# ccalantzis/BRDF

Measured on AMD Instinct MI355X. Metric: BRDF residual-evals/sec (1 M samples, Ward 3-param), whole job; rel-err vs CPU levmar in `parity`, higher is better.
Workload: dtype f64

## Files before the change

### brdf_amd/csrc/brdf_models.h

```cpp
#pragma once

#include <math.h>

#include "lm_machine.h"

namespace brdf {

constexpr double kPi = 3.1415926535897932384626433832795;

enum ModelId : int { MODEL_PHONG = 0, MODEL_BLINN_PHONG = 1, MODEL_WARD = 2, MODEL_COUNT = 3 };

struct Lin {
  double a, b;
};
struct Nl {
  double u0, u1;
};
struct Prep {
  double q1, q2;
};

template <int MODEL>
struct BrdfModel;

// ... 115 lines not shown
  Nl n0;
  Lin lp[kM];
  Lin lm[kM];
  Nl np2, nm2;
  double dinv[kM];
  Lin lq;
  Nl nq;
  Lin lk[kMaxCand];
  Nl nk[kMaxCand];
  double dp[kM], dp_l2, scal;
  double an[2];
  int central, ncand, analytic;

  LM_HD void build(const Request<kM> &r, bool need_base = true, bool analytic_jac = false) {
    ncand = 0;
    analytic = analytic_jac ? 1 : 0;
    if (r.kind == RQ_EVAL_MULTI) {
      ncand = r.nk;
      for (int j = 0; j < kMaxCand; ++j)
        if (j < r.nk) {
          lk[j] = Mdl::lin(r.pk[j]);
          nk[j] = Mdl::nl(r.pk[j]);
        }
      return;
    }
    if (r.kind != RQ_DIF_UPDATE && (need_base || r.kind != RQ_DIF_TRIAL)) {
      l0 = Mdl::lin(r.p);
      n0 = Mdl::nl(r.p);
    }
    central = r.central;
    scal = r.scal;
    dp_l2 = r.dp_l2;
    for (int j = 0; j < kM; ++j) dp[j] = r.dp[j];
    if (r.kind == RQ_JAC && analytic_jac) {
      Mdl::an_scalars(r.p, an);
    } else if (r.kind == RQ_JAC || r.kind == RQ_DIF_JAC) {
      for (int j = 0; j < kM; ++j) {
        double pp[kM] = {r.p[0], r.p[1], r.p[2]};
        pp[j] = r.p[j] + r.d[j];
        lp[j] = Mdl::lin(pp);
        if (j == kM - 1) np2 = Mdl::nl(pp);
        double pm[kM] = {r.p[0], r.p[1], r.p[2]};
        pm[j] = r.p[j] - r.d[j];
        lm[j] = Mdl::lin(pm);
        if (j == kM - 1) nm2 = Mdl::nl(pm);
        dinv[j] = (r.central ? 0.5 : 1.0) / r.d[j];
      }
    }
    if (r.kind == RQ_DIF_TRIAL) {
      lq = Mdl::lin(r.q);
      nq = Mdl::nl(r.q);
    }
  }
};

template <int MODEL, bool FAST, class U>
LM_HD double model_value(const U &u, double c0, const Prep &q) {
  using Mdl = BrdfModel<MODEL>;
  return Mdl::combine(u.l0, c0, Mdl::template shape<FAST>(u.n0, c0, q));
}

template <int MODEL, bool FAST>
LM_HD double model_value_k(const PassUniforms<MODEL> &u, int j, double c0, const Prep &q) {
  using Mdl = BrdfModel<MODEL>;
  return Mdl::combine(u.lk[j], c0, Mdl::template shape<FAST>(u.nk[j], c0, q));
}

template <int MODEL, bool FAST, class U>
LM_HD double model_value_q(const U &u, double c0, const Prep &q) {
  using Mdl = BrdfModel<MODEL>;
  return Mdl::combine(u.lq, c0, Mdl::template shape<FAST>(u.nq, c0, q));
}

template <int MODEL, bool FAST, bool CENTRAL, class U>
LM_HD void model_fd_row_t(const U &u, double c0, const Prep &q, bool need_f0, double &f0, double base_or_nan, bool use_base,
                          double *jrow) {
  using Mdl = BrdfModel<MODEL>;
  const double s0 = Mdl::template shape<FAST>(u.n0, c0, q);
  if (need_f0) f0 = Mdl::combine(u.l0, c0, s0);
  const double sp = Mdl::template shape<FAST>(u.np2, c0, q);
  if (!CENTRAL) {
    const double base = use_base ? base_or_nan : f0;
    jrow[0] = (Mdl::combine(u.lp[0], c0, s0) - base) * u.dinv[0];
    jrow[1] = (Mdl::combine(u.lp[1], c0, s0) - base) * u.dinv[1];
    jrow[2] = (Mdl::combine(u.lp[2], c0, sp) - base) * u.dinv[2];
  } else {
    const double sm = Mdl::template shape<FAST>(u.nm2, c0, q);
    jrow[0] = (Mdl::combine(u.lp[0], c0, s0) - Mdl::combine(u.lm[0], c0, s0)) * u.dinv[0];
    jrow[1] = (Mdl::combine(u.lp[1], c0, s0) - Mdl::combine(u.lm[1], c0, s0)) * u.dinv[1];
    jrow[2] = (Mdl::combine(u.lp[2], c0, sp) - Mdl::combine(u.lm[2], c0, sm)) * u.dinv[2];
  }
}
template <int MODEL, bool FAST, class U>
LM_HD void model_fd_row(const U &u, double c0, const Prep &q, bool need_f0, double &f0,
                        double base_or_nan, bool use_base, double *jrow) {
  if (!u.central)
    model_fd_row_t<MODEL, FAST, false>(u, c0, q, need_f0, f0, base_or_nan, use_base, jrow);
  else
    model_fd_row_t<MODEL, FAST, true>(u, c0, q, need_f0, f0, base_or_nan, use_base, jrow);
}

template <int MODEL, bool FAST, class U>
LM_HD void model_an_row(const U &u, double c0, const Prep &q, double &f0, double *jrow) {
  using Mdl = BrdfModel<MODEL>;
  const double s = Mdl::template shape<FAST>(u.n0, c0, q);
  f0 = Mdl::combine(u.l0, c0, s);
// ... 12 lines not shown
```

### brdf_amd/csrc/device_common.h

```cpp
#pragma once

#include <hip/hip_runtime.h>

#include "brdf_models.h"

namespace brdf {

constexpr int kWave = 64;
constexpr int kSums = SumLayout<kM>::MAX;
constexpr int kSlots = kSums + 1;
constexpr int kNL = SumLayout<kM>::NL;

template <int CTRL, int ROW_MASK, int BANK_MASK>
__device__ __forceinline__ double dpp_move(double v, double idv) {
  const int lo = __builtin_amdgcn_update_dpp(__double2loint(idv), __double2loint(v), CTRL, ROW_MASK, BANK_MASK, false);
  const int hi = __builtin_amdgcn_update_dpp(__double2hiint(idv), __double2hiint(v), CTRL, ROW_MASK, BANK_MASK, false);
  return __hiloint2double(hi, lo);
}

struct OpSum {
  static __device__ __forceinline__ double id() { return 0.0; }
  static __device__ __forceinline__ double apply(double a, double b) { return a + b; }
};
struct OpMax {
// ... 100 lines not shown
  r.l0 = scalar_copy(u.l0);
  r.n0 = scalar_copy(u.n0);
  r.analytic = u.analytic;
  r.central = u.central;
  if (u.analytic) {
    r.an[0] = scalar_copy(u.an[0]);
    r.an[1] = scalar_copy(u.an[1]);
  } else {
    for (int j = 0; j < kM; ++j) {
      r.lp[j] = scalar_copy(u.lp[j]);
      r.dinv[j] = scalar_copy(u.dinv[j]);
      if (u.central) r.lm[j] = scalar_copy(u.lm[j]);
    }
    r.np2 = scalar_copy(u.np2);
    if (u.central) r.nm2 = scalar_copy(u.nm2);
  }
  return r;
}

constexpr int kTrialSums = 3 + 2 * kM;

template <class Core, class Cool>
__device__ __forceinline__ void expand_trial_sums_to(const Core &core, const Cool &cool, const double *dpv, const double *sums, double *out) {
  const double s0 = sums[0], a[kM] = {sums[1], sums[2], sums[3]}, b = sums[1 + kM];
  const double d[kM] = {sums[2 + kM], sums[3 + kM], sums[4 + kM]}, te = sums[2 + 2 * kM];
  const double dp[kM] = {dpv[0], dpv[1], dpv[2]};
  out[0] = s0;
  int c = 1;
#pragma unroll
  for (int i = 0; i < kM; ++i)
#pragma unroll
    for (int j = 0; j <= i; ++j, ++c) {
      double v = (i == j) ? cool.diag[i] : core.jtj[i * kM + j];
      v = fma(a[i], dp[j], v);
      v = fma(dp[i], a[j], v);
      out[c] = fma(b * dp[i], dp[j], v);
    }
#pragma unroll
  for (int j = 0; j < kM; ++j) {
    out[1 + kNL + j] = d[j];
    out[1 + kNL + kM + j] = fma(dp[j], te, core.jte[j]);
  }
}
template <class Core, class Cool>
__device__ __forceinline__ void expand_trial_sums(const Core &core, const Cool &cool, const double *dpv, double *sums) {
  double out[SumLayout<kM>::DIF_TRIAL];
  expand_trial_sums_to(core, cool, dpv, sums, out);
#pragma unroll
  for (int j = 0; j < SumLayout<kM>::DIF_TRIAL; ++j) sums[j] = out[j];
}

template <class Machine>
__device__ __forceinline__ bool fused_trial_step_device(const typename Machine::Cold &c, typename Machine::CoreInts &hi, typename Machine::CoreReals &h,
                                                        typename Machine::Cool &cool, Request<kM> &req, const double *sums, const double *dpv) {
  if (hi.phase != Machine::D_AFTER_TRIAL) return false;
  double out[SumLayout<kM>::DIF_TRIAL];
  expand_trial_sums_to(h, cool, dpv, sums, out);
  return Machine::template fused_trial_step<true, true>(c, hi, h, cool, req, out);
}


__host__ __device__ __forceinline__ int slots_of(int kind) {
  switch (kind) {
  case RQ_EVAL:
  case RQ_SCALED:
  case RQ_DIF_INIT: return 1;
  case RQ_JAC: return SumLayout<kM>::JAC;
  case RQ_DIF_JAC:
  case RQ_DIF_UPDATE: return SumLayout<kM>::DIF_JAC;
  case RQ_DIF_TRIAL: return SumLayout<kM>::DIF_TRIAL;
  case RQ_EVAL_MULTI: return kMaxCand;
  default: return 0;
  }
}

__device__ __forceinline__ void acc_normal_eq(const double *j, double e, double *jtj6, double *jte3) {
  jtj6[0] += j[0] * j[0];
  jtj6[1] += j[0] * j[1];
  jtj6[2] += j[1] * j[1];
  jtj6[3] += j[0] * j[2];
  jtj6[4] += j[1] * j[2];
  jtj6[5] += j[2] * j[2];
  jte3[0] += j[0] * e;
  jte3[1] += j[1] * e;
  jte3[2] += j[2] * e;
}

}
```

### brdf_amd/csrc/lm_machine.h

```cpp
#pragma once

#include <float.h>
#include <math.h>

#if defined(__HIPCC__)
#define LM_HD __host__ __device__ __forceinline__
#else
#define LM_HD inline
#endif

namespace brdf {

constexpr double kEpsilon = 1E-12;
constexpr double kOneThird = 0.3333333334;
constexpr int kLsItMax = 150;
constexpr double kLsPow = 2.1;
constexpr double kInitMu = 1E-03;
#ifndef LM_STAMP
#define LM_STAMP(i) do {} while (0)
#endif

#ifndef LM_PHASE_ENTER
#define LM_PHASE_ENTER(X) true
#endif
// ... 312 lines not shown
    c.want_covar = want_covar_;
    h.k = 0;
    h.stop = 0;
    h.nfev = h.njap = h.nlss = 0;
    h.updjac = 0;
    h.updp = 1;
    h.newjac = 0;
    c.refresh = (M >= 10) ? M : 10;
    h.sel_hx = h.sel_j = 0;
    h.mu = h.jte_inf = h.p_l2 = Real(0.0);
    h.p_e2 = cool.init_e2 = h.pdp_e2 = Real(0.0);
    h.dp_l2 = LmLimits<Real>::max();
    c.ret = kLmError;
    for (int i = 0; i < M; ++i) {
      h.p[i] = p0[i];
      h.jte[i] = cool.diag[i] = h.dp[i] = cool.pdp[i] = Real(0.0);
      cool.spec_jte[i] = Real(0.0);
    }
    for (int i = 0; i < M * M; ++i) h.jtj[i] = cool.spec_jtj[i] = c.covar[i] = Real(0.0);
    for (int i = 0; i < kInfoSz; ++i) c.info[i] = Real(0.0);
    clear_req(h, req);
    if (c.n < M) {
      h.phase = D_DONE;
      req.kind = RQ_DONE;
      return;
    }
    req.kind = RQ_DIF_INIT;
    for (int i = 0; i < M; ++i) req.p[i] = h.p[i];
    h.phase = D_INIT_EVAL;
  }

  static LM_HD void clear_req(const CoreInts &h, Request<M, Real> &req) {
    req.kind = RQ_DONE;
    req.central = 0;
    req.sel_hx = h.sel_hx;
    req.sel_j = h.sel_j;
    req.aux = 0;
    req.dp_l2 = Real(0.0);
    req.scal = Real(1.0);
    req.nk = 0;
    for (int i = 0; i < M; ++i) req.p[i] = req.d[i] = req.q[i] = req.dp[i] = Real(0.0);
  }

  static LM_HD void gradient_stats(CoreReals &h, Cool &cool) {
    h.p_l2 = h.jte_inf = Real(0.0);
    for (int i = 0; i < M; ++i) {
      const Real t = lm_abs(h.jte[i]);
      if (h.jte_inf < t) h.jte_inf = t;
      cool.diag[i] = h.jtj[i * M + i];
      h.p_l2 += h.p[i] * h.p[i];
    }
  }

  template <bool ONE_LANE = false, bool MULTI = false>
  static LM_HD bool fused_trial_step(const Cold &c, CoreInts &hi, CoreReals &h, Cool &cool, Request<M, Real> &req, const Real *s) {
    constexpr int NL = SumLayout<M>::NL;
    if (hi.phase != D_AFTER_TRIAL || !c.speculative || hi.stop) return false;
    const Real e2 = s[0], p_e2 = h.p_e2;
    const Real dF = p_e2 - e2;
    Real mu = h.mu;
    Real dL = Real(0.0);
    for (int i = 0; i < M; ++i) dL += h.dp[i] * (mu * h.dp[i] + h.jte[i]);
    int acc = (dL > Real(0.0) && dF > Real(0.0)) ? 1 : 0;
    int ok = (lm_finite(e2) && (hi.updp || dF > 0)) ? 1 : 0;
    if (ONE_LANE) {
      acc = lm_uniform(acc);
      ok = lm_uniform(ok);
    }
    if (!ok) return false;
    Real pn[M], pe2n;
    int nu, updp;
    if (acc) {
      Real t = (Real(2.0) * dF / dL - Real(1.0));
      t = Real(1.0) - t * t * t;
      mu = mu * ((t >= Real(kOneThird)) ? t : Real(kOneThird));
      nu = 2;
      for (int i = 0; i < M; ++i) pn[i] = cool.pdp[i];
      pe2n = e2;
      updp = 1;
    } else {
      mu *= hi.nu;
      nu = (int)((unsigned)hi.nu << 1);
      if (nu <= hi.nu) return false;
      for (int i = 0; i < M; ++i) pn[i] = h.p[i];
      pe2n = p_e2;
      updp = hi.updp;
    }
    const int k1 = hi.k + 1, updjac1 = hi.updjac + 1;
    if (!(k1 < c.itmax) || k1 == 0) return false;
    if ((updp && nu > 16) || updjac1 == c.refresh) return false;
    const int chain1 = MULTI ? 0 : hi.chain;
    if (MULTI && c.multi > 1 && updp == 0 && chain1 >= 1 && !hi.single) return false;
    const Real *g = s + 1 + NL + (acc ? 0 : M);
    Real A[M * M], b[M], diag[M];
    unpack_lower<M>(s + 1, A);
    Real p_l2 = Real(0.0), jte_inf = Real(0.0);
    for (int i = 0; i < M; ++i) {
      b[i] = g[i];
      const Real t = lm_abs(b[i]);
      if (jte_inf < t) jte_inf = t;
      diag[i] = A[i * M + i];
      p_l2 += pn[i] * pn[i];
    }
    ok = (!(pe2n <= c.o.eps3) && !(jte_inf <= c.o.eps1)) ? 1 : 0;
    if (ONE_LANE) ok = lm_uniform(ok);
    if (!ok) return false;
    Real Am[M * M], dpn[M], pdpn[M];
    for (int i = 0; i < M * M; ++i) Am[i] = A[i];
    for (int i = 0; i < M; ++i) Am[i * M + i] += mu;
    ok = lu_solve<M>(Am, b, dpn);
    Real dp_l2 = Real(0.0);
    for (int i = 0; i < M; ++i) {
      const Real t = dpn[i];
      pdpn[i] = pn[i] + t;
      dp_l2 += t * t;
    }
    ok = (ok && !(dp_l2 <= c.o.eps2sq * p_l2) && !(dp_l2 >= (p_l2 + c.o.eps2) / (Real(kEpsilon) * Real(kEpsilon)))) ? 1 : 0;
    if (ONE_LANE) ok = lm_uniform(ok);
    if (!ok) return false;
    hi.k = k1;
    hi.nu = nu;
    ++hi.nfev;
    ++hi.nlss;
    hi.updjac = updjac1;
    hi.updp = updp;
    hi.newjac = 0;
    if (acc) hi.sel_hx ^= 1;
    hi.sel_j ^= 1;
    hi.accepted = acc;
    if (MULTI) hi.chain = hi.single = 0;
    h.mu = mu;
    h.p_e2 = pe2n;
    h.jte_inf = jte_inf;
    h.p_l2 = p_l2;
    h.dp_l2 = dp_l2;
    h.pdp_e2 = e2;
    for (int i = 0; i < M * M; ++i) {
      h.jtj[i] = Am[i];
      cool.spec_jtj[i] = A[i];
    }
    for (int i = 0; i < M; ++i) {
      h.p[i] = pn[i];
      h.jte[i] = b[i];
      h.dp[i] = dpn[i];
      cool.diag[i] = diag[i];
      cool.pdp[i] = pdpn[i];
      cool.spec_jte[i] = b[i];
    }
    clear_req(hi, req);
    req.kind = RQ_DIF_TRIAL;
    for (int i = 0; i < M; ++i) {
      req.p[i] = pn[i];
      req.q[i] = pdpn[i];
      req.dp[i] = dpn[i];
    }
    req.dp_l2 = dp_l2;
    return true;
  }

  template <bool ONE_LANE = false, bool MULTI = false>
  LM_HD void step(const Real *s, Real maxabs) { run<ONE_LANE, MULTI>(c, h, h.cool, h.req, s, maxabs); }

  template <bool ONE_LANE, bool MULTI = false>
  static LM_HD void run(Cold &c, Core &h, Cool &cool, Request<M, Real> &req, const Real *s, Real maxabs) {
    run<ONE_LANE, MULTI>(c, static_cast<CoreInts &>(h), static_cast<CoreReals &>(h), cool, req, s, maxabs);
  }
  template <bool ONE_LANE, bool MULTI = false>
  static LM_HD void run(Cold &c, CoreInts &hi, CoreReals &h, Cool &cool, Request<M, Real> &req, const Real *s, Real ) {
    int ph = ONE_LANE ? lm_uniform(hi.phase) : hi.phase;
    LM_STAMP(0);
    for (;;) {
      if (ONE_LANE) ph = lm_uniform(ph);
// ... 1345 lines not shown
```

### brdf_amd/csrc/resident_fit_impl.h

```cpp
#pragma once
#include <type_traits>

#if defined(BRDF_STAMPS)
#include <hip/hip_runtime.h>
static __device__ long long g_rlm_stamps[8];
static __device__ long long g_rlm_last;
#endif
#if defined(BRDF_STAMPS) && defined(__HIP_DEVICE_COMPILE__)
#define LM_STAMP(i) do { if (blockIdx.x == 0) { const long long now_ = clock64(); if ((i) != 0) g_rlm_stamps[i] += now_ - g_rlm_last; g_rlm_last = now_; } } while (0)
#endif
#include "batch_fit.h"
#include "stream_fit.h"

namespace brdf {

constexpr int kRThreads = 512;
constexpr int kRSpt = 8;
constexpr int kRTile = kRThreads * kRSpt;
constexpr int kRCap = kRTile;
constexpr int kRowWords = 2 * kSlots;
constexpr int kRowStride = 256;
constexpr int kRedCols = kRThreads / 4;
constexpr long long kSpinBudgetTicks = 200000000LL;

// ... 40 lines not shown
  jtj6[1] = fma(j[0], j[1], jtj6[1]);
  jtj6[2] = fma(j[1], j[1], jtj6[2]);
  jtj6[3] = fma(j[0], j[2], jtj6[3]);
  jtj6[4] = fma(j[1], j[2], jtj6[4]);
  jtj6[5] = fma(j[2], j[2], jtj6[5]);
  jte3[0] = fma(j[0], e, jte3[0]);
  jte3[1] = fma(j[1], e, jte3[1]);
  jte3[2] = fma(j[2], e, jte3[2]);
}
__device__ __forceinline__ double div_by(double x, double d, double r) {
  const double q = x * r;
  return fma(fma(-q, d, x), r, q);
}

#ifdef BRDF_STAMPS
#define RSTAMP(i) do { const long long now_ = clock64(); st_[i] += now_ - last_; last_ = now_; } while (0)
#define RTRACE(ctx_, epoch_, slot_, val_) do { if ((ctx_).trace && (int)(epoch_) == (ctx_).trace_epoch && (threadIdx.x & 63) == 0) (ctx_).trace[blockIdx.x * 8 + (slot_)] = (long long)(val_); } while (0)
#else
#define RSTAMP(i) do {} while (0)
#define RTRACE(ctx_, epoch_, slot_, val_) do {} while (0)
#endif

constexpr int kFc0 = 0, kFx = 1, kFq1 = 2, kFq2 = 3, kFhx = 4, kFwrk = 5, kFtb = 6;
template <int METHOD>
constexpr int sample_fields() { return METHOD == 0 ? 7 : 4; }

template <int METHOD>
struct RegSamples {
  static constexpr bool kUnrolled = true;
  double v[sample_fields<METHOD>()][kRSpt];
  __device__ __forceinline__ double get(int f, int k) const { return v[f][k]; }
  __device__ __forceinline__ void set(int f, int k, double x) { v[f][k] = x; }
};
template <int METHOD>
struct LdsSamples {
  static constexpr bool kUnrolled = false;
  double *base;
  __device__ __forceinline__ double get(int f, int k) const { return base[(f * kRSpt + k) * kWave]; }
  __device__ __forceinline__ void set(int f, int k, double x) { base[(f * kRSpt + k) * kWave] = x; }
};

template <bool UNROLLED, class F>
__device__ __forceinline__ void for_samples(int nk, F &&f) {
  if constexpr (UNROLLED) {
#pragma unroll
    for (int k = 0; k < kRSpt; ++k)
      if (k < nk) f(k);
  } else {
#pragma unroll 2
    for (int k = 0; k < nk; ++k) f(k);
  }
}

template <int NS, bool MAX = true>
__device__ __forceinline__ void worker_reduce(const double *acc, double mx, double *buf, double *out, long long *st_, long long &last_) {
  const int lane = threadIdx.x & (kWave - 1);
  const int wave = threadIdx.x >> 6;
  double v[NS + 1];
#pragma unroll
  for (int k = 0; k < NS; ++k) {
    double t = acc[k];
    t = t + dpp_move<0x111, 0xf, 0xf>(t, 0.0);
    t = t + dpp_move<0x112, 0xf, 0xf>(t, 0.0);
    v[k] = t;
  }
  if constexpr (MAX) {
    double t = mx;
    t = fmax(t, dpp_move<0x111, 0xf, 0xf>(t, 0.0));
    t = fmax(t, dpp_move<0x112, 0xf, 0xf>(t, 0.0));
    v[NS] = t;
  }
  constexpr int NV = NS + (MAX ? 1 : 0);
  if ((threadIdx.x & 3) == 3) {
#pragma unroll
    for (int k = 0; k < NV; ++k) buf[k * kRedCols + (threadIdx.x >> 2)] = v[k];
  }
  __syncthreads();
  RSTAMP(6);
  {
    constexpr int NW = kRThreads / kWave;
    const int k0 = wave, k1 = wave + NW;
    const bool has0 = k0 < NV, has1 = k1 < NV;
    double s0 = 0.0, s1 = 0.0;
    if (has0) {
      const double *src = buf + k0 * kRedCols;
      s0 = (k0 < NS || !MAX) ? src[lane] + src[lane + kWave] : fmax(src[lane], src[lane + kWave]);
    }
    if (has1) {
      const double *src = buf + k1 * kRedCols;
      s1 = (k1 < NS || !MAX) ? src[lane] + src[lane + kWave] : fmax(src[lane], src[lane + kWave]);
    }
    const bool max0 = MAX && has0 && k0 == NS, max1 = MAX && has1 && k1 == NS;
    if (!max0 && !max1) {
      wave_reduce2_to_last<OpSum, OpSum>(s0, s1);
    } else if (max1) {
      wave_reduce2_to_last<OpSum, OpMax>(s0, s1);
    } else {
      wave_reduce2_to_last<OpMax, OpSum>(s0, s1);
    }
    if (lane == kWave - 1) {
      if (has0) out[max0 ? kSums : k0] = s0;
      if (has1) out[max1 ? kSums : k1] = s1;
    }
  }
  __syncthreads();
}

constexpr int kGroup = 16;
constexpr int kMaxGroups = 16;
constexpr int kReplicas = 8;
constexpr size_t kBlockGranules = (size_t)kRowWords * kGroup;
constexpr size_t kRowsGranules = 2 * (size_t)kMaxGroups * kBlockGranules;
constexpr size_t kGroupsGranules = 2 * (size_t)kReplicas * kBlockGranules;

typedef unsigned int u32x4 __attribute__((ext_vector_type(4)));
constexpr int kCacheSc1 = 16;
__device__ __forceinline__ __amdgpu_buffer_rsrc_t table_rsrc(const u64 *p, size_t granules) {
  return __builtin_amdgcn_make_buffer_rsrc(const_cast<u64 *>(p), 0, (int)(granules * sizeof(u64)), 0x00027000);
}
__device__ __forceinline__ void put_cell(__amdgpu_buffer_rsrc_t t, unsigned cell, unsigned tag, double v) {
  const u32x4 d = {(unsigned)__double2loint(v), tag, (unsigned)__double2hiint(v), tag};
  __builtin_amdgcn_raw_buffer_store_b128(d, t, (int)(cell * 16u), 0, kCacheSc1);
}

template <int NS, bool MAX = true>
__device__ __forceinline__ constexpr bool slot_used(int v) { return v < NS || (MAX && v == kSums); }

template <int NS, bool MAX = true, class Ctx>
__device__ __forceinline__ bool gather_block(const Ctx &ctx, __amdgpu_buffer_rsrc_t t, unsigned first, unsigned tag, int ncols,
                                             double (&val)[4], unsigned *polls) {
  const int lane = threadIdx.x & (kWave - 1);
  const int col = lane & 15, r = lane >> 4;
  const long long t0 = (long long)wall_clock64();
  for (unsigned spins = 0;; ++spins) {
    u32x4 d[4];
    bool ready = true;
#pragma unroll
    for (int j = 0; j < 4; ++j) {
      d[j] = u32x4{0u, tag, 0u, tag};
      if ((4 * j < NS) || (MAX && 4 * j <= kSums && kSums < 4 * j + 4)) {
        const int v = 4 * j + r;
        if (slot_used<NS, MAX>(v) && col < ncols) d[j] = __builtin_amdgcn_raw_buffer_load_b128(t, (int)((first + v * kGroup + col) * 16u), 0, kCacheSc1);
      }
    }
#pragma unroll
    for (int j = 0; j < 4; ++j) ready = ready && d[j].y == tag && d[j].w == tag;
    if (__all(ready)) {
#pragma unroll
      for (int j = 0; j < 4; ++j) val[j] = __hiloint2double((int)d[j].z, (int)d[j].x);
      *polls = spins;
      return true;
    }
    if ((spins & 63u) == 63u) {
      if (__hip_atomic_load(&ctx.ctl->abort, __ATOMIC_RELAXED, __HIP_MEMORY_SCOPE_AGENT) == ctx.launch_id ||
          (long long)wall_clock64() - t0 > ctx.spin_ticks) {
        __hip_atomic_store(&ctx.ctl->abort, ctx.launch_id, __ATOMIC_RELAXED, __HIP_MEMORY_SCOPE_AGENT);
        return false;
      }
    }
    __builtin_amdgcn_s_sleep(1);
  }
}

template <int NS, bool MAX>
__device__ __forceinline__ void fold_block(double (&val)[4]) {
  const int r = (int)(threadIdx.x & (kWave - 1)) >> 4;
  double mx = 0.0;
  if constexpr (MAX) mx = row_reduce_to_last<OpMax>(val[kSums / 4]);
#pragma unroll
  for (int j = 0; j < 4; ++j)
    if ((4 * j < NS) || (MAX && j == kSums / 4)) val[j] = row_reduce_to_last<OpSum>(val[j]);
  if (MAX && r == (kSums & 3)) val[kSums / 4] = mx;
}

template <int NS, bool MAX = true, class Ctx>
__device__ __forceinline__ bool control_exchange(const Ctx &ctx, unsigned epoch, double *sums, int *s_abort,
                                                 long long *st_, long long &last_) {
  const int lane = threadIdx.x & (kWave - 1);
  const int col = lane & 15, r = lane >> 4;
  const int G = gridDim.x;
  const int grp = blockIdx.x / kGroup, ngrp = (G + kGroup - 1) / kGroup;
  const int members = min(kGroup, G - grp * kGroup);
  const int leader = grp * kGroup + (grp & 7) % members;
  const unsigned tag = ctx.tag_base + epoch + 1u;
  constexpr unsigned kBlockCells = kSlots * kGroup;
  const __amdgpu_buffer_rsrc_t rows = table_rsrc(ctx.rows, kRowsGranules), groups = table_rsrc(ctx.groups, kGroupsGranules);
  const unsigned my_rows = ((epoch & 1u) * kMaxGroups + grp) * kBlockCells;
  const unsigned my_groups = (epoch & 1u) * kReplicas * kBlockCells;
  const bool withhold = (int)epoch == ctx.sabotage_epoch && blockIdx.x == gridDim.x - 1;
  if (slot_used<NS, MAX>(lane) && lane <= kSums && !withhold) put_cell(rows, my_rows + lane * kGroup + blockIdx.x % kGroup, tag, sums[lane]);

  double val[4];
  unsigned polls = 0;
  if ((int)blockIdx.x == leader) {
    if (!gather_block<NS, MAX>(ctx, rows, my_rows, tag, members, val, &polls)) {
      *s_abort = 1;
      return false;
    }
#ifndef BRDF_TRACE_WORKERS
    RTRACE(ctx, epoch, 6, polls + 1);
#endif
    fold_block<NS, MAX>(val);
#pragma unroll
    for (int j = 0; j < 4; ++j) {
      const double t = dpp_move<0x15F, 0xf, 0xf>(val[j], 0.0);
      const int v = 4 * j + r;
      if (slot_used<NS, MAX>(v) && col < ctx.replicas) put_cell(groups, my_groups + col * kBlockCells + v * kGroup + grp, tag, t);
    }
  }
  RSTAMP(2);
  RTRACE(ctx, epoch, 3, wall_clock64());
  if (!gather_block<NS, MAX>(ctx, groups, my_groups + (blockIdx.x % ctx.replicas) * kBlockCells, tag, ngrp, val, &polls)) {
    *s_abort = 1;
    return false;
  }
  fold_block<NS, MAX>(val);
#pragma unroll
  for (int j = 0; j < 4; ++j) {
    const int v = 4 * j + r;
    if (slot_used<NS, MAX>(v) && col == kGroup - 1) sums[v] = val[j];
  }
  __builtin_amdgcn_fence(__ATOMIC_RELEASE, "wavefront");
  __builtin_amdgcn_wave_barrier();
  RSTAMP(3);
  RTRACE(ctx, epoch, 4, wall_clock64());
#ifndef BRDF_TRACE_WORKERS
  RTRACE(ctx, epoch, 7, polls);
#endif
  return true;
}

template <int MODEL>
__device__ __forceinline__ void build_uniforms_wave(PassUniforms<MODEL> &u, const Request<kM> &r, bool need_base, bool analytic_jac) {
  using Mdl = BrdfModel<MODEL>;
  const int lane = (int)(threadIdx.x & (kWave - 1));
  if (r.kind == RQ_EVAL_MULTI) {
    u.ncand = r.nk;
    u.analytic = analytic_jac ? 1 : 0;
    if (lane < kMaxCand && lane < r.nk) {
      const double pk[kM] = {r.pk[lane][0], r.pk[lane][1], r.pk[lane][2]};
      u.lk[lane] = Mdl::lin(pk);
      u.nk[lane] = Mdl::nl(pk);
    }
// ... 207 lines not shown
      struct TrialUniforms {
        Lin lq;
        Nl nq;
        double dp[kM], dp_l2;
      };
      TrialUniforms tu;
      tu.lq = scalar_copy(u.lq);
      tu.nq = scalar_copy(u.nq);
#pragma unroll
      for (int j = 0; j < kM; ++j) tu.dp[j] = scalar_copy(u.dp[j]);
      tu.dp_l2 = scalar_copy(u.dp_l2);
      const double dpp_s[kM] = {scalar_copy(dpp[0]), scalar_copy(dpp[1]), scalar_copy(dpp[2])};
      const TrialUniforms &u = tu;
      const double *dpp = dpp_s;
      const double rinv = 1.0 / u.dp_l2;
      auto value_q = [&](int k) { return model_value_q<MODEL, FAST>(u, st.get(kFc0, k), prep(k)); };
      auto body = [&](int k, const double w) {
        const int s = k * kRThreads + tid;
        const double h = st.get(kFhx, k), x = st.get(kFx, k);
        double jo[kM] = {jl[s], jl[kRCap + s], jl[2 * kRCap + s]};
        if (pend) {
          const double tp = st.get(kFtb, k);
#pragma unroll
          for (int j = 0; j < kM; ++j) jo[j] = fma(tp, dpp[j], jo[j]);
          jl[s] = jo[0];
          jl[kRCap + s] = jo[1];
          jl[2 * kRCap + s] = jo[2];
        }
        double t = jo[0] * u.dp[0], jn[kM];
        t = fma(jo[1], u.dp[1], t);
        t = fma(jo[2], u.dp[2], t);
        t = div_by(w - h - t, u.dp_l2, rinv);
#pragma unroll
        for (int j = 0; j < kM; ++j) jn[j] = fma(t, u.dp[j], jo[j]);
        double en = x - w, eo = x - h;
        if (dead(k)) en = eo = jn[0] = jn[1] = jn[2] = t = 0.0;
        st.set(kFwrk, k, w);
        st.set(kFtb, k, t);
        acc[0] = fma(en, en, acc[0]);
#pragma unroll
        for (int j = 0; j < kM; ++j) acc[1 + j] = fma(jo[j], t, acc[1 + j]);
        acc[1 + kM] = fma(t, t, acc[1 + kM]);
#pragma unroll
        for (int j = 0; j < kM; ++j) acc[2 + kM + j] = fma(jn[j], en, acc[2 + kM + j]);
        acc[2 + 2 * kM] = fma(t, eo, acc[2 + 2 * kM]);
      };
      for_samples<U>(nk, [&](int k) { body(k, value_q(k)); });
    }
    break;
  default: break;
  }
}

template <int METHOD>
__device__ __forceinline__ void reduce_pass(int kind, const double *acc, double mx, double *red, double *sums, long long *st_, long long &last_) {
  if constexpr (METHOD == 0) {
    switch (kind) {
    case RQ_DIF_JAC: worker_reduce<SumLayout<kM>::DIF_JAC, false>(acc, mx, red, sums, st_, last_); break;
    case RQ_DIF_TRIAL: worker_reduce<kTrialSums, false>(acc, mx, red, sums, st_, last_); break;
    case RQ_EVAL_MULTI: worker_reduce<kMaxCand, false>(acc, mx, red, sums, st_, last_); break;
    default: worker_reduce<1, false>(acc, mx, red, sums, st_, last_); break;
    }
  } else {
    switch (kind) {
    case RQ_JAC: worker_reduce<SumLayout<kM>::JAC, false>(acc, mx, red, sums, st_, last_); break;
    case RQ_EVAL_MULTI: worker_reduce<kMaxCand, false>(acc, mx, red, sums, st_, last_); break;
    default: worker_reduce<1, METHOD == 1>(acc, mx, red, sums, st_, last_); break;
    }
  }
}

#define RESIDENT_KERNEL_HEAD                                      \
  template <int MODEL, int METHOD, bool FAST, bool BATCHED>       \
  __global__ __launch_bounds__(kRThreads) void resident_fit_kernel(ResidentCtx ctx, BatchCtx bctx)
#define RESIDENT_KERNEL_FLAGS constexpr bool RAGGED = false;
#define RESIDENT_KERNEL_COUNT(fit_, stride_) (stride_)
#include "resident_fit_kernel.inc"
#undef RESIDENT_KERNEL_HEAD
#undef RESIDENT_KERNEL_FLAGS
#undef RESIDENT_KERNEL_COUNT

#define RESIDENT_KERNEL_HEAD                          \
  template <int MODEL, int METHOD, bool FAST>         \
  __global__ __launch_bounds__(kRThreads) void resident_fit_ragged_kernel(ResidentCtx ctx, RaggedBatchCtx bctx)
#define RESIDENT_KERNEL_FLAGS constexpr bool BATCHED = true, RAGGED = true;
#define RESIDENT_KERNEL_COUNT(fit_, stride_) ragged_count(bctx.counts, (fit_), (stride_))
#include "resident_fit_kernel.inc"
#undef RESIDENT_KERNEL_HEAD
#undef RESIDENT_KERNEL_FLAGS
#undef RESIDENT_KERNEL_COUNT

using ResidentKernelFn = void (*)(ResidentCtx, BatchCtx);
using ResidentRaggedFn = void (*)(ResidentCtx, RaggedBatchCtx);
constexpr int kFastPath = 0, kExactPath = 1;
struct ResidentKernels {
  ResidentKernelFn single[2], batched[2];
  ResidentRaggedFn ragged[2];
#ifdef BRDF_STAMPS
  void (*take_lm_stamps)(long long *out8);
#endif
};

template <int MODEL, int METHOD, bool FAST, bool BATCHED>
constexpr ResidentKernelFn resident_kernel() {
  if constexpr (FAST || MODEL != MODEL_WARD)
    return resident_fit_kernel<MODEL, METHOD, FAST, BATCHED>;
  else
    return nullptr;
}

template <int MODEL, int METHOD, bool FAST>
constexpr ResidentRaggedFn resident_ragged_kernel() {
  if constexpr (FAST || MODEL != MODEL_WARD)
    return resident_fit_ragged_kernel<MODEL, METHOD, FAST>;
  else
    return nullptr;
}

#ifdef BRDF_STAMPS
static void take_lm_stamps(long long *out8) {
// ... 18 lines not shown
```

### brdf_amd/csrc/resident_fit_kernel.inc

```
RESIDENT_KERNEL_HEAD {
  RESIDENT_KERNEL_FLAGS
  using Machine = RMachine<METHOD>;
  using Mdl = BrdfModel<MODEL>;
  constexpr int NF = sample_fields<METHOD>();
  constexpr bool kControlFromLds = (METHOD == 0) || (METHOD == 1 && !BATCHED);
  static_assert(sizeof(Machine) % 4 == 0, "machine copied as dwords");
  __shared__ Machine sm;
  __shared__ PassUniforms<MODEL> su;
  __shared__ double red[kSlots * kRedCols];
  __shared__ double sums[kSlots];
  __shared__ double dp_prev[kM + 1];
  __shared__ int s_abort, s_bad;
  __shared__ double cst[kControlFromLds ? NF * kRSpt * kWave : 2];
  constexpr int kJl = (METHOD == 0) ? 3 * kRCap : 2;
  __shared__ double jl[kJl];

  const int tid = threadIdx.x;
  const int wave = __builtin_amdgcn_readfirstlane((int)threadIdx.x >> 6);
  const int G = BATCHED ? 1 : (int)gridDim.x;
  const int fit = blockIdx.x;
  const int stride = BATCHED ? bctx.n : ctx.n;
  const int n = RESIDENT_KERNEL_COUNT(fit, stride);
  if constexpr (BATCHED && !FAST) {
    if (bctx.flags[fit] != kNeedsExact) return;
// ... 45 lines not shown
    if constexpr (METHOD == 1)
      su.build(sm.h.req, true, sm.c.analytic_jac != 0);
    else
      su.build(sm.h.req, true, METHOD == 2);
  }

  int vb = BATCHED ? 0 : (int)blockIdx.x;
  if (!BATCHED && (G & 7) == 0) vb = (blockIdx.x & 7) * (G >> 3) + (blockIdx.x >> 3);
  const int tile = (n + G - 1) / G;
  const int begin = vb * tile;
  const int end = min(n, begin + tile);
  const double *pc0 = BATCHED ? bctx.angles + (size_t)fit * 3 * stride : ctx.c0;
  const double *pc1 = BATCHED ? pc0 + stride : ctx.c1;
  const double *pc2 = BATCHED ? pc0 + 2 * (size_t)stride : ctx.c2;
  const double *px = BATCHED ? bctx.x + (size_t)fit * stride : ctx.x;
  const int nk = (tile + kRThreads - 1) / kRThreads;
  const int nfull = max(end - begin, 0) / kRThreads;
  RegSamples<METHOD> rs;
  LdsSamples<METHOD> ls{cst + (tid & (kWave - 1))};
  unsigned okm = 0;
  {
    bool bad = false;
#pragma unroll
    for (int k = 0; k < kRSpt; ++k) {
      const int i = begin + tid + k * kRThreads;
      const bool ok = i < end;
      okm |= ok ? (1u << k) : 0u;
      const int ii = ok ? i : begin;
      const double r0 = pc0[ii];
      const double r1 = Mdl::uses_c1 ? pc1[ii] : 0.0;
      const double r2 = Mdl::uses_c2 ? pc2[ii] : 0.0;
      const Prep q = Mdl::template prepare<FAST>(r0, r1, r2);
      rs.v[kFc0][k] = r0;
      rs.v[kFx][k] = px[ii];
      rs.v[kFq1][k] = q.q1;
      rs.v[kFq2][k] = q.q2;
      if constexpr (METHOD == 0) rs.v[kFhx][k] = rs.v[kFwrk][k] = rs.v[kFtb][k] = 0.0;
      if (FAST && ok && !Mdl::domain_ok(r0, r1, r2)) bad = true;
    }
    if constexpr (BATCHED) {
      if (FAST && bad) s_bad = 1;
    } else {
      if (FAST && bad) __hip_atomic_store(&ctx.ctl->domain_bad, ctx.launch_id, __ATOMIC_RELAXED, __HIP_MEMORY_SCOPE_AGENT);
    }
    if (kControlFromLds && wave == 0) {
#pragma unroll
      for (int f = 0; f < NF; ++f)
#pragma unroll
        for (int k = 0; k < kRSpt; ++k) ls.set(f, k, rs.v[f][k]);
    }
  }
  __syncthreads();

  int cur_sel_hx = 0, cur_sel_j = 0;
  auto decisions = [&](auto &st, bool &pend) {
    pend = false;
    if constexpr (METHOD == 0) {
      pend = sm.h.req.sel_j != cur_sel_j;
      if (pend && sm.h.req.kind != RQ_DIF_TRIAL) pend = false;
      cur_sel_j = sm.h.req.sel_j;
      if (sm.h.req.sel_hx != cur_sel_hx) {
        for_samples<std::remove_reference<decltype(st)>::type::kUnrolled>(nk, [&](int k) { st.set(kFhx, k, st.get(kFwrk, k)); });
        cur_sel_hx = sm.h.req.sel_hx;
      }
    }
  };

  if (wave == 0) {
    long long st_[8] = {0, 0, 0, 0, 0, 0, 0, 0};
    long long last_ = clock64();
    long long n_jac = 0;
    typename Machine::Cold cold0;
    typename std::conditional<METHOD == 0, typename DifMachine<kM>::CoreInts, int>::type ints_regs{};
    if constexpr (METHOD == 0) {
      cold0.itmax = lm_uniform(sm.c.itmax);
      cold0.n = lm_uniform(sm.c.n);
      cold0.want_covar = lm_uniform(sm.c.want_covar);
      cold0.refresh = lm_uniform(sm.c.refresh);
      cold0.speculative = lm_uniform(sm.c.speculative);
      cold0.multi = lm_uniform(sm.c.multi);
      cold0.o.forward = lm_uniform(sm.c.o.forward);
      cold0.o.tau = scalar_copy(sm.c.o.tau);
      cold0.o.eps1 = scalar_copy(sm.c.o.eps1);
      cold0.o.eps2 = scalar_copy(sm.c.o.eps2);
      cold0.o.eps2sq = scalar_copy(sm.c.o.eps2sq);
      cold0.o.eps3 = scalar_copy(sm.c.o.eps3);
      cold0.o.delta = scalar_copy(sm.c.o.delta);
      ints_regs = sm.h;
      Machine::uniform_ints(ints_regs);
    }
    const int fused = (METHOD == 0) ? (BATCHED ? bctx.dif_fused : ctx.dif_fused) : 0;
    int n_fused = 0;
    (void)cold0, (void)ints_regs, (void)fused;
    const long long t_first = (long long)wall_clock64();
    unsigned epoch = 0;
    for (;; ++epoch) {
      const int kind = sm.h.req.kind;
      if (kind == RQ_DONE) break;
      if (kind == RQ_JAC || kind == RQ_DIF_JAC) ++n_jac;
      RTRACE(ctx, epoch, 0, wall_clock64());
      {
        bool pend;
        double acc[kSums];
#pragma unroll
        for (int k = 0; k < kSums; ++k) acc[k] = 0.0;
        double mx = 0.0;
        const double dpp[kM] = {dp_prev[0], dp_prev[1], dp_prev[2]};
        if constexpr (kControlFromLds) {
          decisions(ls, pend);
          sweep_pass<MODEL, METHOD, FAST>(kind, su, ls, jl, tid, nk, nfull, okm, pend, dpp, acc, mx);
        } else {
          decisions(rs, pend);
          sweep_pass<MODEL, METHOD, FAST>(kind, su, rs, jl, tid, nk, nfull, okm, pend, dpp, acc, mx);
        }
        RSTAMP(5);
        RTRACE(ctx, epoch, 1, wall_clock64());
        reduce_pass<METHOD>(kind, acc, mx, red, sums, st_, last_);
      }
      RSTAMP(1);
      RTRACE(ctx, epoch, 2, wall_clock64());
      bool alive = true;
      if constexpr (BATCHED && FAST) {
        if (epoch == 0) {
          if (s_bad) {
            if (tid == 0) bctx.flags[fit] = kNeedsExact;
            s_abort = 1;
            alive = false;
          } else if (tid == 0) {
            bctx.flags[fit] = 0;
          }
        }
      }
      if constexpr (!BATCHED) {
       if (gridDim.x > 1) {
        if constexpr (METHOD == 0) {
          switch (kind) {
          case RQ_DIF_JAC: alive = control_exchange<SumLayout<kM>::DIF_JAC, false>(ctx, epoch, sums, &s_abort, st_, last_); break;
          case RQ_DIF_TRIAL: alive = control_exchange<kTrialSums, false>(ctx, epoch, sums, &s_abort, st_, last_); break;
          case RQ_EVAL_MULTI: alive = control_exchange<kMaxCand, false>(ctx, epoch, sums, &s_abort, st_, last_); break;
          default: alive = control_exchange<1, false>(ctx, epoch, sums, &s_abort, st_, last_); break;
          }
        } else {
          switch (kind) {
          case RQ_JAC: alive = control_exchange<SumLayout<kM>::JAC, false>(ctx, epoch, sums, &s_abort, st_, last_); break;
          case RQ_EVAL_MULTI: alive = control_exchange<kMaxCand, false>(ctx, epoch, sums, &s_abort, st_, last_); break;
          default: alive = control_exchange<1, METHOD == 1>(ctx, epoch, sums, &s_abort, st_, last_); break;
          }
        }
       }
      }
      if (!alive) {
        __syncthreads();
        return;
      }
      bool stepped = false;
      if (kind == RQ_DIF_TRIAL) {
        if constexpr (METHOD == 0) {
          if (fused) {
            stepped = fused_trial_step_device<Machine>(cold0, ints_regs, static_cast<typename Machine::CoreReals &>(sm.h), sm.h.cool, sm.h.req, sums, su.dp);
            if (stepped) {
              ++n_fused;
              Machine::uniform_ints(ints_regs);
            }
          }
          if (!stepped) expand_trial_sums(static_cast<const typename Machine::Core &>(sm.h), sm.h.cool, su.dp, sums);
        }
#pragma unroll
        for (int j = 0; j < kM; ++j) dp_prev[j] = su.dp[j];
        dp_prev[kM] = su.dp_l2;
      }
      if (!stepped) {
        if constexpr (METHOD == 0) {
          typename Machine::Cold cc;
          cc.itmax = cold0.itmax, cc.n = cold0.n, cc.want_covar = cold0.want_covar, cc.refresh = cold0.refresh;
          cc.speculative = cold0.speculative, cc.multi = cold0.multi, cc.o = cold0.o;
          for (int i = 0; i < kInfoSz; ++i) cc.info[i] = 0.0;
          for (int i = 0; i < kM * kM; ++i) cc.covar[i] = 0.0;
          cc.ret = kLmError;
          Machine::template run<true, true>(cc, ints_regs, static_cast<typename Machine::CoreReals &>(sm.h), sm.h.cool, sm.h.req, sums, sums[kSums]);
          Machine::uniform_ints(ints_regs);
          if (sm.h.req.kind == RQ_DONE) {
            for (int i = 0; i < kInfoSz; ++i) sm.c.info[i] = cc.info[i];
            for (int i = 0; i < kM * kM; ++i) sm.c.covar[i] = cc.covar[i];
            sm.c.ret = cc.ret;
          }
        } else
        if constexpr (METHOD == 1)
          sm.template step<true, true, false, !BATCHED>(sums, sums[kSums]);
        else
          sm.template step<true>(sums, sums[kSums]);
      }
      RSTAMP(7);
      if (sm.h.req.kind != RQ_DONE) {
        if constexpr (METHOD == 1 && !BATCHED)
          build_uniforms_wave(su, sm.h.req, false, sm.c.analytic_jac != 0);
        else if constexpr (METHOD == 1)
          su.build(sm.h.req, false, sm.c.analytic_jac != 0);
        else
          su.build(sm.h.req, false, METHOD == 2);
      }
      RTRACE(ctx, epoch, 5, wall_clock64());
      __syncthreads();
      RSTAMP(4);
    }
    if constexpr (BATCHED) {
      if constexpr (RAGGED && FAST) {
        if (epoch == 0 && tid == 0) bctx.flags[fit] = 0;
      }
      if (tid == 0) {
        double *po = bctx.p + (size_t)fit * kM;
        for (int i = 0; i < kM; ++i) po[i] = sm.h.p[i];
        if (bctx.info)
          for (int i = 0; i < kInfoSz; ++i) bctx.info[(size_t)fit * kInfoSz + i] = sm.c.info[i];
        if (bctx.ret) bctx.ret[fit] = sm.c.ret;
      }
      return;
    }
    if (blockIdx.x == 0 && tid == 0) {
      Mailbox *mb = ctx.mbox;
      mb->ret = sm.c.ret;
      mb->passes = (int)epoch;
      if constexpr (METHOD == 1)
        mb->infeasible_mask = sm.c.infeasible_mask;
      else
        mb->infeasible_mask = 0;
      mb->domain_bad = __hip_atomic_load(&ctx.ctl->domain_bad, __ATOMIC_RELAXED, __HIP_MEMORY_SCOPE_AGENT) == ctx.launch_id ? 1 : 0;
      mb->n_jac = n_jac;
      mb->n_eval = (long long)epoch - n_jac;
      mb->t_first = t_first;
      mb->t_last = (long long)wall_clock64();
      st_[0] = n_fused;
      for (int k = 0; k < 8; ++k) mb->stamps[k] = st_[k];
      for (int i = 0; i < kM; ++i) mb->p[i] = sm.h.p[i];
      for (int i = 0; i < kInfoSz; ++i) mb->info[i] = sm.c.info[i];
      for (int i = 0; i < kM * kM; ++i) mb->covar[i] = sm.c.covar[i];
      __threadfence_system();
      __hip_atomic_store(&mb->done, 1, __ATOMIC_RELEASE, __HIP_MEMORY_SCOPE_SYSTEM);
    }
    return;
  }

  long long wst_[8] = {0, 0, 0, 0, 0, 0, 0, 0}, wlast_ = 0;
#ifdef BRDF_TRACE_WORKERS
  unsigned wepoch = 0;
#endif
  for (;;) {
    const int kind = sm.h.req.kind;
    if (kind == RQ_DONE) break;
    bool pend;
    decisions(rs, pend);
    double acc[kSums];
#pragma unroll
    for (int k = 0; k < kSums; ++k) acc[k] = 0.0;
    double mx = 0.0;
    const double dpp[kM] = {dp_prev[0], dp_prev[1], dp_prev[2]};
    sweep_pass<MODEL, METHOD, FAST>(kind, su, rs, jl, tid, nk, nfull, okm, pend, dpp, acc, mx);
#ifdef BRDF_TRACE_WORKERS
    if constexpr (!BATCHED) {
      if (wave == 4) RTRACE(ctx, wepoch, 6, wall_clock64());
      if (wave == 7) RTRACE(ctx, wepoch, 7, wall_clock64());
      ++wepoch;
    }
#endif
    reduce_pass<METHOD>(kind, acc, mx, red, sums, wst_, wlast_);
    __syncthreads();
    if (s_abort) return;
  }
}
```

Before: 136.8 billion.

## Publish per-wave reduced sums directly to cross-block table and build trial uniforms from registers

```diff
diff --git a/brdf_amd/csrc/brdf_models.h b/brdf_amd/csrc/brdf_models.h
--- a/brdf_amd/csrc/brdf_models.h
+++ b/brdf_amd/csrc/brdf_models.h
@@ -191,6 +191,17 @@
       nq = Mdl::nl(r.q);
     }
   }
+
+  LM_HD void build_trial(const double *q, const double *dpv, double dpl2, bool analytic_jac = false) {
+    ncand = 0;
+    analytic = analytic_jac ? 1 : 0;
+    central = 0;
+    scal = 1.0;
+    dp_l2 = dpl2;
+    for (int j = 0; j < kM; ++j) dp[j] = dpv[j];
+    lq = Mdl::lin(q);
+    nq = Mdl::nl(q);
+  }
 };
 
 template <int MODEL, bool FAST, class U>
diff --git a/brdf_amd/csrc/device_common.h b/brdf_amd/csrc/device_common.h
--- a/brdf_amd/csrc/device_common.h
+++ b/brdf_amd/csrc/device_common.h
@@ -176,11 +176,12 @@
 
 template <class Machine>
 __device__ __forceinline__ bool fused_trial_step_device(const typename Machine::Cold &c, typename Machine::CoreInts &hi, typename Machine::CoreReals &h,
-                                                        typename Machine::Cool &cool, Request<kM> &req, const double *sums, const double *dpv) {
+                                                        typename Machine::Cool &cool, Request<kM> &req, const double *sums, const double *dpv,
+                                                        typename Machine::NextTrial *next = nullptr) {
   if (hi.phase != Machine::D_AFTER_TRIAL) return false;
   double out[SumLayout<kM>::DIF_TRIAL];
   expand_trial_sums_to(h, cool, dpv, sums, out);
-  return Machine::template fused_trial_step<true, true>(c, hi, h, cool, req, out);
+  return Machine::template fused_trial_step<true, true>(c, hi, h, cool, req, out, next);
 }
 
 
diff --git a/brdf_amd/csrc/lm_machine.h b/brdf_amd/csrc/lm_machine.h
--- a/brdf_amd/csrc/lm_machine.h
+++ b/brdf_amd/csrc/lm_machine.h
@@ -388,8 +388,12 @@
     }
   }
 
+  struct NextTrial {
+    Real q[M], dp[M], dp_l2;
+  };
   template <bool ONE_LANE = false, bool MULTI = false>
-  static LM_HD bool fused_trial_step(const Cold &c, CoreInts &hi, CoreReals &h, Cool &cool, Request<M, Real> &req, const Real *s) {
+  static LM_HD bool fused_trial_step(const Cold &c, CoreInts &hi, CoreReals &h, Cool &cool, Request<M, Real> &req, const Real *s,
+                                     NextTrial *next = nullptr) {
     constexpr int NL = SumLayout<M>::NL;
     if (hi.phase != D_AFTER_TRIAL || !c.speculative || hi.stop) return false;
     const Real e2 = s[0], p_e2 = h.p_e2;
@@ -454,6 +458,13 @@
     ok = (ok && !(dp_l2 <= c.o.eps2sq * p_l2) && !(dp_l2 >= (p_l2 + c.o.eps2) / (Real(kEpsilon) * Real(kEpsilon)))) ? 1 : 0;
     if (ONE_LANE) ok = lm_uniform(ok);
     if (!ok) return false;
+    if (next) {
+      for (int i = 0; i < M; ++i) {
+        next->q[i] = pdpn[i];
+        next->dp[i] = dpn[i];
+      }
+      next->dp_l2 = dp_l2;
+    }
     hi.k = k1;
     hi.nu = nu;
     ++hi.nfev;
diff --git a/brdf_amd/csrc/resident_fit_impl.h b/brdf_amd/csrc/resident_fit_impl.h
--- a/brdf_amd/csrc/resident_fit_impl.h
+++ b/brdf_amd/csrc/resident_fit_impl.h
@@ -116,8 +116,34 @@
   }
 }
 
-template <int NS, bool MAX = true>
-__device__ __forceinline__ void worker_reduce(const double *acc, double mx, double *buf, double *out, long long *st_, long long &last_) {
+constexpr int kGroup = 16;
+constexpr int kMaxGroups = 16;
+constexpr int kReplicas = 8;
+constexpr size_t kBlockGranules = (size_t)kRowWords * kGroup;
+constexpr size_t kRowsGranules = 2 * (size_t)kMaxGroups * kBlockGranules;
+constexpr size_t kGroupsGranules = 2 * (size_t)kReplicas * kBlockGranules;
+
+typedef unsigned int u32x4 __attribute__((ext_vector_type(4)));
+constexpr int kCacheSc1 = 16;
+__device__ __forceinline__ __amdgpu_buffer_rsrc_t table_rsrc(const u64 *p, size_t granules) {
+  return __builtin_amdgcn_make_buffer_rsrc(const_cast<u64 *>(p), 0, (int)(granules * sizeof(u64)), 0x00027000);
+}
+__device__ __forceinline__ void put_cell(__amdgpu_buffer_rsrc_t t, unsigned cell, unsigned tag, double v) {
+  const u32x4 d = {(unsigned)__double2loint(v), tag, (unsigned)__double2hiint(v), tag};
+  __builtin_amdgcn_raw_buffer_store_b128(d, t, (int)(cell * 16u), 0, kCacheSc1);
+}
+
+struct RowPublish {
+  const u64 *rows;
+  unsigned cell0;
+  unsigned tag;
+  bool on;
+  bool withhold;
+};
+
+template <int NS, bool MAX = true, bool PUB = false>
+__device__ __forceinline__ void worker_reduce(const double *acc, double mx, double *buf, double *out, const RowPublish &pub, long long *st_,
+                                              long long &last_) {
   const int lane = threadIdx.x & (kWave - 1);
   const int wave = threadIdx.x >> 6;
   double v[NS + 1];
@@ -162,6 +188,16 @@
     } else {
       wave_reduce2_to_last<OpMax, OpSum>(s0, s1);
     }
+    if constexpr (PUB) {
+      if (pub.on) {
+        if (lane == kWave - 1 && !pub.withhold) {
+          const __amdgpu_buffer_rsrc_t rows = table_rsrc(pub.rows, kRowsGranules);
+          if (has0) put_cell(rows, pub.cell0 + (max0 ? kSums : k0) * kGroup, pub.tag, s0);
+          if (has1) put_cell(rows, pub.cell0 + (max1 ? kSums : k1) * kGroup, pub.tag, s1);
+        }
+        return;
+      }
+    }
     if (lane == kWave - 1) {
       if (has0) out[max0 ? kSums : k0] = s0;
       if (has1) out[max1 ? kSums : k1] = s1;
@@ -170,21 +206,10 @@
   __syncthreads();
 }
 
-constexpr int kGroup = 16;
-constexpr int kMaxGroups = 16;
-constexpr int kReplicas = 8;
-constexpr size_t kBlockGranules = (size_t)kRowWords * kGroup;
-constexpr size_t kRowsGranules = 2 * (size_t)kMaxGroups * kBlockGranules;
-constexpr size_t kGroupsGranules = 2 * (size_t)kReplicas * kBlockGranules;
-
-typedef unsigned int u32x4 __attribute__((ext_vector_type(4)));
-constexpr int kCacheSc1 = 16;
-__device__ __forceinline__ __amdgpu_buffer_rsrc_t table_rsrc(const u64 *p, size_t granules) {
-  return __builtin_amdgcn_make_buffer_rsrc(const_cast<u64 *>(p), 0, (int)(granules * sizeof(u64)), 0x00027000);
-}
-__device__ __forceinline__ void put_cell(__amdgpu_buffer_rsrc_t t, unsigned cell, unsigned tag, double v) {
-  const u32x4 d = {(unsigned)__double2loint(v), tag, (unsigned)__double2hiint(v), tag};
-  __builtin_amdgcn_raw_buffer_store_b128(d, t, (int)(cell * 16u), 0, kCacheSc1);
+__device__ __forceinline__ RowPublish row_publish(const ResidentCtx &ctx, unsigned epoch) {
+  const unsigned grp = blockIdx.x / kGroup;
+  return RowPublish{ctx.rows, ((epoch & 1u) * kMaxGroups + grp) * (kSlots * kGroup) + blockIdx.x % kGroup, ctx.tag_base + epoch + 1u, gridDim.x > 1,
+                    (int)epoch == ctx.sabotage_epoch && blockIdx.x == gridDim.x - 1};
 }
 
 template <int NS, bool MAX = true>
@@ -237,7 +262,7 @@
   if (MAX && r == (kSums & 3)) val[kSums / 4] = mx;
 }
 
-template <int NS, bool MAX = true, class Ctx>
+template <int NS, bool MAX = true, bool PUBLISHED = false, class Ctx>
 __device__ __forceinline__ bool control_exchange(const Ctx &ctx, unsigned epoch, double *sums, int *s_abort,
                                                  long long *st_, long long &last_) {
   const int lane = threadIdx.x & (kWave - 1);
@@ -251,8 +276,10 @@
   const __amdgpu_buffer_rsrc_t rows = table_rsrc(ctx.rows, kRowsGranules), groups = table_rsrc(ctx.groups, kGroupsGranules);
   const unsigned my_rows = ((epoch & 1u) * kMaxGroups + grp) * kBlockCells;
   const unsigned my_groups = (epoch & 1u) * kReplicas * kBlockCells;
-  const bool withhold = (int)epoch == ctx.sabotage_epoch && blockIdx.x == gridDim.x - 1;
-  if (slot_used<NS, MAX>(lane) && lane <= kSums && !withhold) put_cell(rows, my_rows + lane * kGroup + blockIdx.x % kGroup, tag, sums[lane]);
+  if constexpr (!PUBLISHED) {
+    const bool withhold = (int)epoch == ctx.sabotage_epoch && blockIdx.x == gridDim.x - 1;
+    if (slot_used<NS, MAX>(lane) && lane <= kSums && !withhold) put_cell(rows, my_rows + lane * kGroup + blockIdx.x % kGroup, tag, sums[lane]);
+  }
 
   double val[4];
   unsigned polls = 0;
@@ -566,20 +593,21 @@
   }
 }
 
-template <int METHOD>
-__device__ __forceinline__ void reduce_pass(int kind, const double *acc, double mx, double *red, double *sums, long long *st_, long long &last_) {
+template <int METHOD, bool PUB = false>
+__device__ __forceinline__ void reduce_pass(int kind, const double *acc, double mx, double *red, double *sums, const RowPublish &pub, long long *st_,
+                                            long long &last_) {
   if constexpr (METHOD == 0) {
     switch (kind) {
-    case RQ_DIF_JAC: worker_reduce<SumLayout<kM>::DIF_JAC, false>(acc, mx, red, sums, st_, last_); break;
-    case RQ_DIF_TRIAL: worker_reduce<kTrialSums, false>(acc, mx, red, sums, st_, last_); break;
-    case RQ_EVAL_MULTI: worker_reduce<kMaxCand, false>(acc, mx, red, sums, st_, last_); break;
-    default: worker_reduce<1, false>(acc, mx, red, sums, st_, last_); break;
+    case RQ_DIF_JAC: worker_reduce<SumLayout<kM>::DIF_JAC, false, PUB>(acc, mx, red, sums, pub, st_, last_); break;
+    case RQ_DIF_TRIAL: worker_reduce<kTrialSums, false, PUB>(acc, mx, red, sums, pub, st_, last_); break;
+    case RQ_EVAL_MULTI: worker_reduce<kMaxCand, false, PUB>(acc, mx, red, sums, pub, st_, last_); break;
+    default: worker_reduce<1, false, PUB>(acc, mx, red, sums, pub, st_, last_); break;
     }
   } else {
     switch (kind) {
-    case RQ_JAC: worker_reduce<SumLayout<kM>::JAC, false>(acc, mx, red, sums, st_, last_); break;
-    case RQ_EVAL_MULTI: worker_reduce<kMaxCand, false>(acc, mx, red, sums, st_, last_); break;
-    default: worker_reduce<1, METHOD == 1>(acc, mx, red, sums, st_, last_); break;
+    case RQ_JAC: worker_reduce<SumLayout<kM>::JAC, false, PUB>(acc, mx, red, sums, pub, st_, last_); break;
+    case RQ_EVAL_MULTI: worker_reduce<kMaxCand, false, PUB>(acc, mx, red, sums, pub, st_, last_); break;
+    default: worker_reduce<1, METHOD == 1, PUB>(acc, mx, red, sums, pub, st_, last_); break;
     }
   }
 }
diff --git a/brdf_amd/csrc/resident_fit_kernel.inc b/brdf_amd/csrc/resident_fit_kernel.inc
--- a/brdf_amd/csrc/resident_fit_kernel.inc
+++ b/brdf_amd/csrc/resident_fit_kernel.inc
@@ -121,6 +121,13 @@
   }
   __syncthreads();
 
+  constexpr bool kPub = !BATCHED;
+  auto row_pub = [&](unsigned epoch) {
+    if constexpr (kPub)
+      return row_publish(ctx, epoch);
+    else
+      return RowPublish{nullptr, 0u, 0u, false, false};
+  };
   int cur_sel_hx = 0, cur_sel_j = 0;
   auto decisions = [&](auto &st, bool &pend) {
     pend = false;
@@ -184,7 +191,7 @@
         }
         RSTAMP(5);
         RTRACE(ctx, epoch, 1, wall_clock64());
-        reduce_pass<METHOD>(kind, acc, mx, red, sums, st_, last_);
+        reduce_pass<METHOD, kPub>(kind, acc, mx, red, sums, row_pub(epoch), st_, last_);
       }
       RSTAMP(1);
       RTRACE(ctx, epoch, 2, wall_clock64());
@@ -204,16 +211,16 @@
        if (gridDim.x > 1) {
         if constexpr (METHOD == 0) {
           switch (kind) {
-          case RQ_DIF_JAC: alive = control_exchange<SumLayout<kM>::DIF_JAC, false>(ctx, epoch, sums, &s_abort, st_, last_); break;
-          case RQ_DIF_TRIAL: alive = control_exchange<kTrialSums, false>(ctx, epoch, sums, &s_abort, st_, last_); break;
-          case RQ_EVAL_MULTI: alive = control_exchange<kMaxCand, false>(ctx, epoch, sums, &s_abort, st_, last_); break;
-          default: alive = control_exchange<1, false>(ctx, epoch, sums, &s_abort, st_, last_); break;
+          case RQ_DIF_JAC: alive = control_exchange<SumLayout<kM>::DIF_JAC, false, kPub>(ctx, epoch, sums, &s_abort, st_, last_); break;
+          case RQ_DIF_TRIAL: alive = control_exchange<kTrialSums, false, kPub>(ctx, epoch, sums, &s_abort, st_, last_); break;
+          case RQ_EVAL_MULTI: alive = control_exchange<kMaxCand, false, kPub>(ctx, epoch, sums, &s_abort, st_, last_); break;
+          default: alive = control_exchange<1, false, kPub>(ctx, epoch, sums, &s_abort, st_, last_); break;
           }
         } else {
           switch (kind) {
-          case RQ_JAC: alive = control_exchange<SumLayout<kM>::JAC, false>(ctx, epoch, sums, &s_abort, st_, last_); break;
-          case RQ_EVAL_MULTI: alive = control_exchange<kMaxCand, false>(ctx, epoch, sums, &s_abort, st_, last_); break;
-          default: alive = control_exchange<1, METHOD == 1>(ctx, epoch, sums, &s_abort, st_, last_); break;
+          case RQ_JAC: alive = control_exchange<SumLayout<kM>::JAC, false, kPub>(ctx, epoch, sums, &s_abort, st_, last_); break;
+          case RQ_EVAL_MULTI: alive = control_exchange<kMaxCand, false, kPub>(ctx, epoch, sums, &s_abort, st_, last_); break;
+          default: alive = control_exchange<1, METHOD == 1, kPub>(ctx, epoch, sums, &s_abort, st_, last_); break;
           }
         }
        }
@@ -223,10 +230,14 @@
         return;
       }
       bool stepped = false;
+      constexpr bool kTrialFromRegs = METHOD == 0 && !BATCHED;
+      typename std::conditional<METHOD == 0, typename DifMachine<kM>::NextTrial, int>::type next_trial{};
+      (void)next_trial;
       if (kind == RQ_DIF_TRIAL) {
         if constexpr (METHOD == 0) {
           if (fused) {
-            stepped = fused_trial_step_device<Machine>(cold0, ints_regs, static_cast<typename Machine::CoreReals &>(sm.h), sm.h.cool, sm.h.req, sums, su.dp);
+            stepped = fused_trial_step_device<Machine>(cold0, ints_regs, static_cast<typename Machine::CoreReals &>(sm.h), sm.h.cool, sm.h.req, sums, su.dp,
+                                                       kTrialFromRegs ? &next_trial : nullptr);
             if (stepped) {
               ++n_fused;
               Machine::uniform_ints(ints_regs);
@@ -260,7 +271,9 @@
           sm.template step<true>(sums, sums[kSums]);
       }
       RSTAMP(7);
-      if (sm.h.req.kind != RQ_DONE) {
+      if (kTrialFromRegs && stepped) {
+        if constexpr (METHOD == 0) su.build_trial(next_trial.q, next_trial.dp, next_trial.dp_l2, false);
+      } else if (sm.h.req.kind != RQ_DONE) {
         if constexpr (METHOD == 1 && !BATCHED)
           build_uniforms_wave(su, sm.h.req, false, sm.c.analytic_jac != 0);
         else if constexpr (METHOD == 1)
@@ -310,10 +323,7 @@
   }
 
   long long wst_[8] = {0, 0, 0, 0, 0, 0, 0, 0}, wlast_ = 0;
-#ifdef BRDF_TRACE_WORKERS
-  unsigned wepoch = 0;
-#endif
-  for (;;) {
+  for (unsigned epoch = 0;; ++epoch) {
     const int kind = sm.h.req.kind;
     if (kind == RQ_DONE) break;
     bool pend;
@@ -326,12 +336,11 @@
     sweep_pass<MODEL, METHOD, FAST>(kind, su, rs, jl, tid, nk, nfull, okm, pend, dpp, acc, mx);
 #ifdef BRDF_TRACE_WORKERS
     if constexpr (!BATCHED) {
-      if (wave == 4) RTRACE(ctx, wepoch, 6, wall_clock64());
-      if (wave == 7) RTRACE(ctx, wepoch, 7, wall_clock64());
-      ++wepoch;
+      if (wave == 4) RTRACE(ctx, epoch, 6, wall_clock64());
+      if (wave == 7) RTRACE(ctx, epoch, 7, wall_clock64());
     }
 #endif
-    reduce_pass<METHOD>(kind, acc, mx, red, sums, wst_, wlast_);
+    reduce_pass<METHOD, kPub>(kind, acc, mx, red, sums, row_pub(epoch), wst_, wlast_);
     __syncthreads();
     if (s_abort) return;
   }
```

Result: faster. 139.9 billion, median of 6 (+2.3%).
